# jtaghia/ciMRGP

Hardware: AMD Instinct MI355X
Metric: GP posteriors/sec at N=8192 (Gram + Cholesky + solve + predictive mean/var) (higher is better)
Workload: dtype f64; 1 GPU; BASELINE configs[1]: 1-D, N=8192 single-resolution single-partition RBF GP per GPU, q=2 outputs, N/4=2048 test points, ell=0.1, sf2=1, noise=0.01; partitions_per_gpu=1, backend=none, rows_queues=2, front_queue=True

## Files before the change

### cimrgp_amd/csrc/gemm_nt.hip

```cpp
#include "common.hpp"
#include "gemm_tile.hpp"

namespace cimrgp {

namespace {

template <typename T, bool LOWER, int W>
__global__ __launch_bounds__(256, 2)
void k_gemm_nt_sub(T* __restrict__ C, int64_t ldc,
                   const T* __restrict__ A, int64_t lda,
                   const T* __restrict__ B, int64_t ldb,
                   int M, int N, int K, int tiles_n, int64_t sc, int64_t sa, int64_t sb, int skip_first)
{
    if (skip_first && blockIdx.x == 0) return;
    constexpr int GT = 32 * W;
    __shared__ __attribute__((aligned(16))) unsigned char smem[4 * GT * LROW];
    C += (int64_t)blockIdx.y * sc;
    A += (int64_t)blockIdx.y * sa;
    B += (int64_t)blockIdx.y * sb;
    int ti, tj;
    if (LOWER) {
        const int id = blockIdx.x;
        ti = (int)((sqrtf(8.0f * (float)id + 1.0f) - 1.0f) * 0.5f);
        while (ti * (ti + 1) / 2 > id) --ti;
        while ((ti + 1) * (ti + 2) / 2 <= id) ++ti;
        tj = id - ti * (ti + 1) / 2;
    } else {
        ti = blockIdx.x / tiles_n;
        tj = blockIdx.x - ti * tiles_n;
    }
    const bool interior = (ti + 1) * GT <= M && (tj + 1) * GT <= N && (K % (KT_BYTES / (int)sizeof(T))) == 0;
    if (interior) gemm_tile<T, LOWER, false, W>(smem, C, ldc, A, lda, B, ldb, M, N, K, ti, tj);
    else          gemm_tile<T, LOWER, true,  W>(smem, C, ldc, A, lda, B, ldb, M, N, K, ti, tj);
}


constexpr int PERS_STRIP = 4;

static __device__ __forceinline__ int pers_div(int q, int d)
{
    int r = (int)((float)q / (float)d);
    r -= (r * d > q);
    r += ((r + 1) * d <= q);
    return r;
}

template <bool LOWER>
static __device__ __forceinline__ void pers_tile_decode(int q, int tiles_m, int tiles_n, int& ti, int& tj)
{
    if (LOWER) {
        static_assert(PERS_STRIP == 4, "closed form below");
        const int sfull = tiles_m >> 2;
        int s, h;
        if (q < 8 * sfull * sfull + 2 * sfull) {
            s = (int)((sqrtf(8.0f * (float)q + 1.0f) - 1.0f) * 0.125f);
            s -= (8 * s * s + 2 * s > q);
            s += (8 * (s + 1) * (s + 1) + 2 * (s + 1) <= q);
            h = 4;
        } else {
            s = sfull;
            h = tiles_m - 4 * sfull;
        }
        const int r0 = 4 * s;
        const int off = q - (8 * s * s + 2 * s);
        if (off < h * r0) {
            tj = (h == 4) ? (off >> 2) : (h == 2) ? (off >> 1) : (h == 1) ? off : (int)(((unsigned)off * 43691u) >> 17);
            ti = r0 + off - tj * h;
        } else {
            int o2 = off - h * r0, c = 0;
            if (o2 >= h) {
                o2 -= h; c = 1;
                if (o2 >= h - 1) {
                    o2 -= h - 1; c = 2;
                    if (o2 >= h - 2) { o2 -= h - 2; c = 3; }
                }
            }
            tj = r0 + c;
            ti = r0 + c + o2;
        }
    } else {
        const int per_strip = PERS_STRIP * tiles_n;
        const int s = pers_div(q, per_strip);
        const int r0 = PERS_STRIP * s;
        const int h = min(PERS_STRIP, tiles_m - r0);
        const int off = q - s * per_strip;
        tj = (h == 4) ? (off >> 2) : (h == 2) ? (off >> 1) : (h == 1) ? off : pers_div(off, 3);
        ti = r0 + off - tj * h;
    }
}

static __device__ __forceinline__ void pers_tile_decode_head_first(int q, int tiles_m, int& ti, int& tj)
{
    if (q < tiles_m - 1) { ti = q + 1; tj = 0; return; }
    q -= tiles_m - 1;
    if (q < tiles_m - 1) { ti = q + 1; tj = 1; return; }
    q -= tiles_m - 1;
    pers_tile_decode<true>(q, tiles_m - 2, 0, ti, tj);
    ti += 2;
    tj += 2;
}

static __device__ __forceinline__ int pers_tile_number(int w, int i, int grid, int ntiles)
{
    const int per_xcd = grid >> 3;
    const int x = w & 7, j = w >> 3;
    const int q = (i * 8 + x) * per_xcd + j;
    return q < ntiles ? q : -1;
}

static __device__ __forceinline__ __amdgpu_buffer_rsrc_t tile_rsrc(const void* p)
{
    return __builtin_amdgcn_make_buffer_rsrc(const_cast<void*>(p), 0, 0x7fffffff, 0x00020000);
}
static __device__ __forceinline__ __amdgpu_buffer_rsrc_t tile_rsrc_null(const void* p)
{
    return __builtin_amdgcn_make_buffer_rsrc(const_cast<void*>(p), 0, 0, 0x00020000);
}
typedef unsigned int cbuf_u2 __attribute__((ext_vector_type(2)));
template <typename T> static __device__ __forceinline__ T cbuf_load(__amdgpu_buffer_rsrc_t r, int voff, int soff);
template <> __device__ __forceinline__ double cbuf_load<double>(__amdgpu_buffer_rsrc_t r, int voff, int soff)
{
    const cbuf_u2 v = __builtin_amdgcn_raw_buffer_load_b64(r, voff, soff, 0);
    return __hiloint2double((int)v.y, (int)v.x);
}
template <> __device__ __forceinline__ float cbuf_load<float>(__amdgpu_buffer_rsrc_t r, int voff, int soff)
{
    return __uint_as_float(__builtin_amdgcn_raw_buffer_load_b32(r, voff, soff, 0));
}
template <typename T> static __device__ __forceinline__ void cbuf_store(T v, __amdgpu_buffer_rsrc_t r, int voff, int soff);
template <> __device__ __forceinline__ void cbuf_store<double>(double v, __amdgpu_buffer_rsrc_t r, int voff, int soff)
{
    const cbuf_u2 u = {(unsigned)__double2loint(v), (unsigned)__double2hiint(v)};
    __builtin_amdgcn_raw_buffer_store_b64(u, r, voff, soff, 0);
}
template <> __device__ __forceinline__ void cbuf_store<float>(float v, __amdgpu_buffer_rsrc_t r, int voff, int soff)
{
    __builtin_amdgcn_raw_buffer_store_b32(__float_as_uint(v), r, voff, soff, 0);
}

constexpr int PERS_THREADS = 512;
constexpr int PERS_STAGES = 16;

template <typename T, bool LOWER, int NKT, bool MULTI = false>
__global__ __launch_bounds__(PERS_THREADS)
void k_gemm_nt_pers(T* __restrict__ C, int64_t ldc, const T* __restrict__ A, int64_t lda,
                    const T* __restrict__ B, int64_t ldb, int tiles_m, int tiles_n, int ntiles, int heads, int* __restrict__ flag,
                    int nkc)
{
    static_assert(NKT == 16 || NKT == 8, "sixteen C events per tile: one or two per K stage");
    constexpr int EVS = 16 / NKT;
    using X = Mx<T>;
    using acc_t = typename X::acc_t;
    constexpr int BKE = KT_BYTES / (int)sizeof(T);
    constexpr int GT = 128;
    constexpr int OP_BYTES = GT * LROW;
    constexpr int RS = (sizeof(T) == 8) ? 4 : 1;
    __shared__ __attribute__((aligned(16))) unsigned char smem[4 * OP_BYTES];

    const int tid = threadIdx.x, lane = tid & 63;
    const int wave = __builtin_amdgcn_readfirstlane(tid >> 6);
    const int wr = wave >> 2, wc = wave & 3;
    const int sc = tid & 7, sr = tid >> 3;
    const int grid = (int)gridDim.x, wg = (int)blockIdx.x;

    int a_off_e[2], b_off_e[2];
#pragma unroll
    for (int p = 0; p < 2; ++p) {
        a_off_e[p] = (sr + 64 * p) * (int)lda + sc * X::EPC;
        b_off_e[p] = (sr + 64 * p) * (int)ldb + sc * X::EPC;
    }
    const int frow = lane & 15, fslot = lane >> 4;
    const unsigned a_frag = (unsigned)((wr * 64 + frow) * LROW + fslot * 8);
    const unsigned b_frag = (unsigned)((wc * 32 + frow) * LROW + fslot * 8);
    const int lrow0 = wr * 64 + X::crow(lane, 0), lcol0 = wc * 32 + (lane & 15);
    const int coff = lrow0 * (int)ldc + lcol0;
    const int cbyte0 = coff * (int)sizeof(T);
    const int row_bytes = (int)ldc * (int)sizeof(T);

    auto decode = [&](int q, int& i_, int& j_) {
        if (LOWER && heads > 0) pers_tile_decode_head_first(q, tiles_m, i_, j_);
        else pers_tile_decode<LOWER>(q, tiles_m, tiles_n, i_, j_);
    };
    auto signal_stored = [&]() {
        asm volatile("s_waitcnt vmcnt(0)" ::: "memory");
        __syncthreads();
        if (tid == 0) {
            __builtin_amdgcn_fence(__ATOMIC_RELEASE, "agent");
            asm volatile("s_waitcnt vmcnt(0)" ::: "memory");
            __hip_atomic_fetch_add(flag, 1, __ATOMIC_RELAXED, __HIP_MEMORY_SCOPE_AGENT);
        }
    };
    __shared__ int flag_a[8], flag_b[8];
    if (tid < 8) { flag_a[tid] = -1; flag_b[tid] = -1; }
    int gstage = 0;
#define PERS_POST(flag_)  do { __atomic_signal_fence(__ATOMIC_SEQ_CST);                                                  \
                               __hip_atomic_store(&flag_[wave], gstage, __ATOMIC_RELAXED, __HIP_MEMORY_SCOPE_WORKGROUP);  \
                               __atomic_signal_fence(__ATOMIC_SEQ_CST); } while (0)
#define PERS_PEEK(flag_)  __hip_atomic_load(&flag_[lane & 7], __ATOMIC_RELAXED, __HIP_MEMORY_SCOPE_WORKGROUP)
#define PERS_WAIT(flag_, seen_, g_)                                                                              \
        do {                                                                                                     \
            int v_ = (seen_);                                                                                    \
            while (__builtin_amdgcn_ballot_w64(v_ - (g_) < 0) != 0ull) v_ = PERS_PEEK(flag_);                    \
            __atomic_signal_fence(__ATOMIC_SEQ_CST);                                                             \
        } while (0)
    int it = 0;
    int t = pers_tile_number(wg, it, grid, ntiles);
    if (t < 0) return;
    int ti, tj;
    decode(t, ti, tj);
    int t_nx = pers_tile_number(wg, 1, grid, ntiles), ti_nx = ti, tj_nx = tj;
    if (t_nx >= 0) decode(t_nx, ti_nx, tj_nx);
    bool prev_head = false;
    bool prv_stored = true;
    T* c_cur = C + (int64_t)ti * GT * ldc + (int64_t)tj * GT;
    const T* a_cur = A + (int64_t)ti * GT * lda;
    const T* b_cur = B + (int64_t)tj * GT * ldb;
    T* c_prv = c_cur;
    typedef unsigned int v4u __attribute__((ext_vector_type(4)));
    v4u ra[2], rb[2];
    const v4u sign4 = {0x80000000u, 0x80000000u, 0x80000000u, 0x80000000u};
    uint2 fa[2][4], fb[2][2];
    acc_t acc0[4][2], acc1[4][2];

#define PERS_GLOAD(ap_, bp_, kt_)                                                  \
    {                                                                              \
        _Pragma("unroll") for (int p = 0; p < 2; ++p) {                            \
            ra[p] = *reinterpret_cast<const v4u*>((ap_) + (a_off_e[p] + (kt_) * BKE)); \
            rb[p] = *reinterpret_cast<const v4u*>((bp_) + (b_off_e[p] + (kt_) * BKE)); \
        }                                                                          \
    }
#define PERS_SWRITE(buf_)                                                          \
    {                                                                              \
        unsigned char* as_ = smem + (buf_) * 2 * OP_BYTES;                         \
        unsigned char* bs_ = as_ + OP_BYTES;                                       \
        _Pragma("unroll") for (int p = 0; p < 2; ++p) {                            \
             \
             \
            *reinterpret_cast<v4u*>(as_ + (sr + 64 * p) * LROW + sc * 16) = (sizeof(T) == 4) ? (ra[p] ^ sign4) : ra[p]; \
            *reinterpret_cast<v4u*>(bs_ + (sr + 64 * p) * LROW + sc * 16) = rb[p]; \
        }                                                                          \
    }
#define PERS_FRAGS_NF(set_, buf_, s_)                                              \
    {                                                                              \
        const unsigned char* as_ = smem + (buf_) * 2 * OP_BYTES;                   \
        const unsigned char* bs_ = as_ + OP_BYTES;                                 \
        _Pragma("unroll") for (int mi = 0; mi < 4; ++mi)                           \
            fa[set_][mi] = *reinterpret_cast<const uint2*>(as_ + a_frag + mi * 16 * LROW + (s_) * 32); \
        _Pragma("unroll") for (int ni = 0; ni < 2; ++ni)                           \
            fb[set_][ni] = *reinterpret_cast<const uint2*>(bs_ + b_frag + ni * 16 * LROW + (s_) * 32); \
    }
#define PERS_FRAGS(set_, buf_, s_)  { PERS_FRAGS_NF(set_, buf_, s_) __builtin_amdgcn_sched_barrier(0); }
#define PERS_MMA_NF(cur_, set_)                                                    \
    {                                                                              \
        _Pragma("unroll") for (int mi = 0; mi < 4; ++mi) {                         \
            _Pragma("unroll") for (int ni = 0; ni < 2; ++ni)                       \
                cur_[mi][ni] = (sizeof(T) == 4) ? X::mma(fa[set_][mi], fb[set_][ni], cur_[mi][ni])            \
                                                : X::mma_neg(fa[set_][mi], fb[set_][ni], cur_[mi][ni]);       \
        }                                                                          \
    }
#define PERS_MMA(cur_, set_)  { PERS_MMA_NF(cur_, set_) __builtin_amdgcn_sched_barrier(0); }
#define PERS_INTERLEAVE()                                                          \
    {                                                                              \
        _Pragma("unroll") for (int i_ = 0; i_ < 8; ++i_) {                         \
            __builtin_amdgcn_sched_group_barrier(0x008, 1, 0);                     \
            __builtin_amdgcn_sched_group_barrier(0x096, 6, 0);                     \
        }                                                                          \
        __builtin_amdgcn_sched_barrier(0);                                         \
    }

    PERS_GLOAD(a_cur, b_cur, 0);
#pragma unroll
    for (int mi = 0; mi < 4; ++mi)
#pragma unroll
        for (int ni = 0; ni < 2; ++ni)
#pragma unroll
            for (int r = 0; r < 4; ++r)
                acc0[mi][ni][r] = (c_cur + ((int64_t)(mi * 16 + RS * r) * ldc + ni * 16))[coff];
#pragma unroll
    for (int mi = 0; mi < 4; ++mi)
#pragma unroll
        for (int ni = 0; ni < 2; ++ni) acc1[mi][ni] = acc_zero<T>();
    PERS_SWRITE(0);
    PERS_GLOAD(a_cur, b_cur, 1);
    lds_barrier();
    PERS_FRAGS(0, 0, 0);

#define PERS_EVENT_ONE(oth_, e_)                                                                         \
        {                                                          \
                const int mi_ = (e_) >> 2, ne_ = ((e_) >> 1) & 1, r0_ = 2 * ((e_) & 1);                         \
                 \
                 \
                 \
                const int so0_ = (mi_ * 16 + RS * r0_) * row_bytes + ne_ * 16 * (int)sizeof(T);                 \
                const int so1_ = so0_ + RS * row_bytes;                                                         \
                cbuf_store<T>(oth_[mi_][ne_][r0_], rs_prv, cbyte0, so0_);                                       \
                cbuf_store<T>(oth_[mi_][ne_][r0_ + 1], rs_prv, cbyte0, so1_);                                   \
                              \
                oth_[mi_][ne_][r0_] = cbuf_load<T>(rs_nxt, cbyte0, so0_);                                       \
                oth_[mi_][ne_][r0_ + 1] = cbuf_load<T>(rs_nxt, cbyte0, so1_);                                   \
            }
#define PERS_EVENT_BLOCK(oth_)                                                                                  \
        { _Pragma("unroll") for (int ev_ = 0; ev_ < EVS; ++ev_) { PERS_EVENT_ONE(oth_, kt * EVS + ev_) } }
#define PERS_STAGE_OPERANDS(kt_)                                                                                \
            PERS_SWRITE(((kt_) & 1) ^ 1);                \
            if ((kt_) + 2 < NKT) PERS_GLOAD(a_chk, b_chk, (kt_) + 2)                \
            else                 PERS_GLOAD(a_adv, b_adv, (kt_) + 2 - NKT)
#define PERS_SYNC_TOP()      PERS_WAIT(flag_b, seen_b, gstage - 1);
#define PERS_SYNC_WRITTEN()  PERS_POST(flag_a);
#define PERS_SYNC_READ()     PERS_POST(flag_b); seen_a = PERS_PEEK(flag_a); __builtin_amdgcn_sched_barrier(0);
#define PERS_BARRIER_A()     PERS_WAIT(flag_a, seen_a, gstage)
#define PERS_BARRIER_B()     do { } while (0)
#define PERS_SYNC_PEEK_B()   seen_b = PERS_PEEK(flag_b); __builtin_amdgcn_sched_barrier(0);
#define PERS_SYNC_NEXT()     ++gstage;
#define PERS_PASS(cur_, oth_)                                                                                   \
    {                                                                                                           \
        const int tn_ = t_nx;                                                                                   \
        const bool has_next = tn_ >= 0;                                                                         \
        const int ni_ = has_next ? ti_nx : ti, nj_ = has_next ? tj_nx : tj;                                     \
        const T* c_nxt = C + (int64_t)ni_ * GT * ldc + (int64_t)nj_ * GT;           \
        const __amdgpu_buffer_rsrc_t rs_nxt = tile_rsrc(c_nxt);                                                 \
        const T* a_nxt = A + (int64_t)ni_ * GT * lda;                                                           \
        const T* b_nxt = B + (int64_t)nj_ * GT * ldb;                                                           \
         \
         \
         \
         \
        for (int kc = 0; kc < (MULTI ? nkc : 1); ++kc) {                                                        \
        const bool lastc = !MULTI || (kc + 1 == nkc);                                                           \
        const __amdgpu_buffer_rsrc_t rs_prv = (prv_stored || kc > 0) ? tile_rsrc_null(c_prv) : tile_rsrc(c_prv); \
        const T* a_chk = a_cur + kc * (NKT * BKE);                                                              \
        const T* b_chk = b_cur + kc * (NKT * BKE);                                                              \
        const T* a_adv = lastc ? a_nxt : a_chk + NKT * BKE;                                                     \
        const T* b_adv = lastc ? b_nxt : b_chk + NKT * BKE;                                                     \
        _Pragma("unroll") for (int kt = 0; kt < NKT; ++kt) {                                                    \
            if (kt == NKT / 2 && lastc) {               \
                t_nx = pers_tile_number(wg, it + 2, grid, ntiles);                                              \
                if (t_nx >= 0) decode(t_nx, ti_nx, tj_nx);                                                      \
            }                                                                                                   \
            PERS_SYNC_TOP()                           \
            PERS_STAGE_OPERANDS(kt)                                                                             \
            PERS_SYNC_WRITTEN()                                  \
            PERS_EVENT_BLOCK(oth_)                                                                              \
              \
              \
            PERS_FRAGS_NF(1, kt & 1, 1);                                                                        \
            PERS_MMA_NF(cur_, 0);                                                                               \
            PERS_INTERLEAVE();                                                                                  \
            PERS_FRAGS(0, kt & 1, 2);                                                                           \
            PERS_MMA(cur_, 1);                                                                                  \
            PERS_FRAGS(1, kt & 1, 3);                                                                           \
            PERS_SYNC_READ()                          \
            PERS_MMA(cur_, 0);                                                                                  \
            PERS_BARRIER_A();                                                         \
            PERS_FRAGS(0, (kt & 1) ^ 1, 0);                                  \
            PERS_SYNC_PEEK_B()                        \
            PERS_MMA(cur_, 1);                                                                                  \
            PERS_BARRIER_B();                         \
            PERS_SYNC_NEXT()                                                                                    \
        }                                                                                                       \
        }                                                                                      \
        if (prev_head) signal_stored();               \
        prev_head = (t < heads);                                                                                \
        c_prv = c_cur;                                                                                          \
        if (!has_next) {                                                                                        \
               \
            _Pragma("unroll") for (int mi = 0; mi < 4; ++mi)                                                    \
                _Pragma("unroll") for (int ni = 0; ni < 2; ++ni)                                                \
                    _Pragma("unroll") for (int r = 0; r < 4; ++r)                                               \
                        (c_cur + ((int64_t)(mi * 16 + RS * r) * ldc + ni * 16))[coff] = cur_[mi][ni][r];        \
            if (prev_head) signal_stored();                                                                     \
            return;                                                                                             \
        }                                                                                                       \
        prv_stored = false;                                                                                     \
        t = tn_; ti = ni_; tj = nj_; ++it;                                                                      \
        c_cur = const_cast<T*>(c_nxt); a_cur = a_nxt; b_cur = b_nxt;                                            \
    }

    int seen_a = -1, seen_b = -1;
    for (;;) {
        PERS_PASS(acc0, acc1)
        PERS_PASS(acc1, acc0)
    }
#undef PERS_PASS
#undef PERS_STAGE_OPERANDS
#undef PERS_SYNC_TOP
#undef PERS_SYNC_WRITTEN
#undef PERS_SYNC_READ
#undef PERS_SYNC_PEEK_B
#undef PERS_SYNC_NEXT
#undef PERS_BARRIER_A
#undef PERS_BARRIER_B
#undef PERS_EVENT_BLOCK
#undef PERS_EVENT_ONE
#undef PERS_INTERLEAVE
#undef PERS_MMA
#undef PERS_MMA_NF
#undef PERS_FRAGS_NF
#undef PERS_FRAGS
#undef PERS_SWRITE
#undef PERS_GLOAD
}

constexpr int THIN_RPW = 8;
constexpr int THIN_MAXM = 4;
template <typename T, int M>
__global__ __launch_bounds__(256)
void k_thin_update(T* __restrict__ C, int64_t ldc, const T* __restrict__ A, int64_t lda, const T* __restrict__ B, int64_t ldb,
                   int N, int K, int64_t sc, int64_t sa, int64_t sb)
{
    typedef unsigned int v4u __attribute__((ext_vector_type(4)));
    constexpr int EPL = 32 / (int)sizeof(T);
    constexpr int CH = 64 * EPL;
    C += (int64_t)blockIdx.y * sc;
    A += (int64_t)blockIdx.y * sa;
    B += (int64_t)blockIdx.y * sb;
    const int lane = threadIdx.x & 63, wave = threadIdx.x >> 6;
    const int n0 = ((int)blockIdx.x * 4 + wave) * THIN_RPW;
    if (n0 >= N) return;
    T acc[THIN_RPW][M];
#pragma unroll
    for (int i = 0; i < THIN_RPW; ++i)
#pragma unroll
        for (int r = 0; r < M; ++r) acc[i][r] = (T)0;
    for (int kc = 0; kc < K; kc += CH) {
        const int ke = kc + lane * EPL;
        const bool live = ke < K;
        T av[M][EPL];
#pragma unroll
        for (int r = 0; r < M; ++r) {
            union { v4u v[2]; T t[EPL]; } u;
            u.v[0] = live ? *reinterpret_cast<const v4u*>(A + (int64_t)r * lda + ke) : v4u{0, 0, 0, 0};
            u.v[1] = (live && ke + EPL / 2 < K) ? *reinterpret_cast<const v4u*>(A + (int64_t)r * lda + ke + EPL / 2) : v4u{0, 0, 0, 0};
#pragma unroll
            for (int e = 0; e < EPL; ++e) av[r][e] = u.t[e];
        }
        union { v4u v[2]; T t[EPL]; } bv[THIN_RPW];
#pragma unroll
        for (int i = 0; i < THIN_RPW; ++i) {
            const int n = min(n0 + i, N - 1);
            const T* bp = B + (int64_t)n * ldb + ke;
            bv[i].v[0] = live ? *reinterpret_cast<const v4u*>(bp) : v4u{0, 0, 0, 0};
            bv[i].v[1] = (live && ke + EPL / 2 < K) ? *reinterpret_cast<const v4u*>(bp + EPL / 2) : v4u{0, 0, 0, 0};
        }
#pragma unroll
        for (int i = 0; i < THIN_RPW; ++i)
#pragma unroll
            for (int r = 0; r < M; ++r)
#pragma unroll
                for (int e = 0; e < EPL; ++e) acc[i][r] += av[r][e] * bv[i].t[e];
    }
#pragma unroll
    for (int i = 0; i < THIN_RPW; ++i)
#pragma unroll
        for (int r = 0; r < M; ++r) {
            T v = acc[i][r];
#pragma unroll
            for (int off = 32; off > 0; off >>= 1) v += __shfl_xor(v, off, 64);
            acc[i][r] = v;
        }
    if (lane < THIN_RPW * M) {
        const int i = lane / M, r = lane - i * M;
        T v = (T)0;
#pragma unroll
        for (int ii = 0; ii < THIN_RPW; ++ii)
#pragma unroll
            for (int rr = 0; rr < M; ++rr)
                if (ii == i && rr == r) v = acc[ii][rr];
        if (n0 + i < N) C[(int64_t)r * ldc + n0 + i] -= v;
    }
}

}

template <typename T, int W>
static int gemm_launch(T* c, int64_t ldc, const T* a, int64_t lda, const T* b, int64_t ldb,
                       int64_t m, int64_t n, int k, bool lower, hipStream_t st, const GemmBatch& bt)
{
    const char* fn = "gemm_nt_sub";
    constexpr int GT = 32 * W;
    const int64_t tm = (m + GT - 1) / GT, tn = (n + GT - 1) / GT;
    const int64_t tiles = lower ? tm * (tm + 1) / 2 : tm * tn;
    CIMRGP_REQUIRE(tiles < (1ll << 31), fn, "grid too large");
    CIMRGP_REQUIRE(bt.count >= 1 && bt.count < 65536, fn, "batch count out of range");
    const dim3 grid((unsigned)tiles, (unsigned)bt.count);
    if (lower) hipLaunchKernelGGL((k_gemm_nt_sub<T, true, W>), grid, dim3(256), 0, st,
                                  c, ldc, a, lda, b, ldb, (int)m, (int)n, k, (int)tn, bt.sc, bt.sa, bt.sb, bt.skip_first);
    else       hipLaunchKernelGGL((k_gemm_nt_sub<T, false, W>), grid, dim3(256), 0, st,
                                  c, ldc, a, lda, b, ldb, (int)m, (int)n, k, (int)tn, bt.sc, bt.sa, bt.sb, bt.skip_first);
    CIMRGP_LAUNCH_CHECK(fn);
    return 0;
}

int gemm_pers_head_tiles(int64_t m, int k, int elem_bytes)
{
    if (elem_bytes != 8) return 0;
    const int bke = KT_BYTES / elem_bytes;
    if (knobs().gemm_pers < 8 || m % 128 != 0 || m / 128 < 3 || k % bke != 0 || k / bke != PERS_STAGES) return 0;
    return (int)(2 * (m / 128) - 2);
}

bool gemm_uses_tile64(int64_t m, int64_t n, bool lower, int count)
{
    const int64_t t128 = ((m + 127) / 128) * ((n + 127) / 128) / (lower ? 2 : 1) * count;
    const int64_t t64 = ((m + 63) / 64) * ((n + 63) / 64) / (lower ? 2 : 1) * count;
    const int64_t thin = (m < n) ? m : n;
    return !lower && t64 >= 32 && thin > 32 && (t128 < 768 || thin <= 64);
}

template <typename T>
int gemm_nt_sub(T* c, int64_t ldc, const T* a, int64_t lda, const T* b, int64_t ldb,
                int64_t m, int64_t n, int k, bool lower, hipStream_t st, GemmBatch bt)
{
    const char* fn = "gemm_nt_sub";
    if (m <= 0 || n <= 0 || k <= 0) return 0;
    CIMRGP_REQUIRE(m < (1ll << 30) && n < (1ll << 30), fn, "matrix too large");
    CIMRGP_REQUIRE(aligned16(a) && aligned16(b), fn, "operand base not 16-byte aligned");
    CIMRGP_REQUIRE(lda % Mx<T>::EPC == 0 && ldb % Mx<T>::EPC == 0, fn, "leading dimension not a multiple of 16 bytes");
    CIMRGP_REQUIRE(!lower || m == n, fn, "lower update needs a square C");
    if (!lower && m <= THIN_MAXM && !bt.skip_first && !bt.head_first && k % Mx<T>::EPC == 0 && aligned16(a) && aligned16(b)) {
        const dim3 grid((unsigned)((n + 4 * THIN_RPW - 1) / (4 * THIN_RPW)), (unsigned)bt.count);
#define CIMRGP_THIN(M_) case M_: hipLaunchKernelGGL((k_thin_update<T, M_>), grid, dim3(256), 0, st, c, ldc, a, lda, b, ldb, (int)n, k, bt.sc, bt.sa, bt.sb); break;
        switch ((int)m) { CIMRGP_THIN(1) CIMRGP_THIN(2) CIMRGP_THIN(3) CIMRGP_THIN(4) }
#undef CIMRGP_THIN
        CIMRGP_LAUNCH_CHECK(fn);
        return 0;
    }
    CIMRGP_REQUIRE(!bt.skip_first || gemm_uses_tile64(m, n, lower, bt.count), fn, "skip_first needs a 64-tile launch");
    const int64_t t128 = ((m + 127) / 128) * ((n + 127) / 128) / (lower ? 2 : 1) * bt.count;
    const int64_t t64 = ((m + 63) / 64) * ((n + 63) / 64) / (lower ? 2 : 1) * bt.count;
    if constexpr (sizeof(T) == 8) {
        constexpr int bke = KT_BYTES / (int)sizeof(T);
        const int want = (bt.pers >= 0) ? bt.pers : knobs().gemm_pers;
        const int nkt = (k % bke) ? 0 : k / bke;
        constexpr int pers_nkt = PERS_STAGES;
        const int nkc = (nkt > 0 && nkt % pers_nkt == 0) ? nkt / pers_nkt : 0;
        if (want >= 8 && nkc >= 1 && nkc <= knobs().pers_max_chunks && (nkc == 1 || !bt.head_first) &&
            bt.count == 1 && !bt.skip_first && m % 128 == 0 && n % 128 == 0 &&
            ldc < (1ll << 20) && lda < (1ll << 23) && ldb < (1ll << 23) && (t128 >= knobs().pers_min_tiles || bt.head_first || bt.pers_force)) {
            const int64_t tm = m / 128, tn = n / 128;
            const int heads = (bt.head_first && lower && tm >= 3) ? (int)(2 * tm - 2) : 0;
            CIMRGP_REQUIRE(!bt.head_first || heads > 0, fn, "a head-first update needs a lower update of at least 3 x 3 tiles");
            const int64_t tiles = (lower ? tm * (tm + 1) / 2 : tm * tn) - (heads ? 1 : 0);
            const int cus = (want < 256 ? want : 256) & ~7;
            const int64_t rounds = (tiles + cus - 1) / cus;
            int64_t g8 = (tiles + rounds - 1) / rounds;
            g8 = (g8 + 7) / 8 * 8;
            if (g8 > cus) g8 = cus;
            const dim3 grid((unsigned)g8);
#define CIMRGP_PERS_LAUNCH(LOW_, MULTI_) \
            hipLaunchKernelGGL((k_gemm_nt_pers<T, LOW_, pers_nkt, MULTI_>), grid, dim3(PERS_THREADS), 0, st, c, ldc, a, lda, b, ldb, (int)tm, (int)tn, (int)tiles, heads, bt.flag, nkc)
            if (lower) { if (nkc > 1) CIMRGP_PERS_LAUNCH(true, true); else CIMRGP_PERS_LAUNCH(true, false); }
            else       { if (nkc > 1) CIMRGP_PERS_LAUNCH(false, true); else CIMRGP_PERS_LAUNCH(false, false); }
#undef CIMRGP_PERS_LAUNCH
            CIMRGP_LAUNCH_CHECK(fn);
            return 0;
        }
    }
    CIMRGP_REQUIRE(!bt.head_first, fn, "head-first update not eligible for the persistent kernel (gemm_pers_eligible)");
    const int64_t thin = (m < n) ? m : n;
    if (!bt.skip_first && thin <= 32) return gemm_launch<T, 1>(c, ldc, a, lda, b, ldb, m, n, k, lower, st, bt);
    if (t64 < 32) return gemm_launch<T, 1>(c, ldc, a, lda, b, ldb, m, n, k, lower, st, bt);
    if (t128 < 768 || thin <= 64) return gemm_launch<T, 2>(c, ldc, a, lda, b, ldb, m, n, k, lower, st, bt);
    return gemm_launch<T, 4>(c, ldc, a, lda, b, ldb, m, n, k, lower, st, bt);
}

template int gemm_nt_sub<double>(double*, int64_t, const double*, int64_t, const double*, int64_t,
                                 int64_t, int64_t, int, bool, hipStream_t, GemmBatch);
template int gemm_nt_sub<float>(float*, int64_t, const float*, int64_t, const float*, int64_t,
                                int64_t, int64_t, int, bool, hipStream_t, GemmBatch);

}
```

Baseline: 147.8 posteriors/s.

## Partition persistent GEMM tiles into contiguous per-XCD regions and stream C traffic

Tile scheduling for the persistent GEMM kernel moves into a shared header. The assignment changes from interleaving tiles round-robin across the eight XCDs to giving each XCD a contiguous range of tiles: column-major rectangular regions for the general case, and head tiles first then contiguous ranges for the lower case. This should keep A/B panel reuse inside each XCD's L2. C loads and stores in the single-chunk case now carry a streaming cache-policy bit so C traffic does not evict operands. A guard on tile count is added for the general path to avoid int overflow in the new index math.

New measurement: 148.5 posteriors/s (median of 6 runs). Within noise of the previous version (+0.5%).

```diff
diff --git a/cimrgp_amd/csrc/gemm_nt.hip b/cimrgp_amd/csrc/gemm_nt.hip
--- a/cimrgp_amd/csrc/gemm_nt.hip
+++ b/cimrgp_amd/csrc/gemm_nt.hip
@@ -1,5 +1,6 @@
 #include "common.hpp"
 #include "gemm_tile.hpp"
+#include "pers_order.hpp"
 
 namespace cimrgp {
 
@@ -35,107 +36,33 @@
 }
 
 
-constexpr int PERS_STRIP = 4;
-
-static __device__ __forceinline__ int pers_div(int q, int d)
-{
-    int r = (int)((float)q / (float)d);
-    r -= (r * d > q);
-    r += ((r + 1) * d <= q);
-    return r;
-}
-
-template <bool LOWER>
-static __device__ __forceinline__ void pers_tile_decode(int q, int tiles_m, int tiles_n, int& ti, int& tj)
-{
-    if (LOWER) {
-        static_assert(PERS_STRIP == 4, "closed form below");
-        const int sfull = tiles_m >> 2;
-        int s, h;
-        if (q < 8 * sfull * sfull + 2 * sfull) {
-            s = (int)((sqrtf(8.0f * (float)q + 1.0f) - 1.0f) * 0.125f);
-            s -= (8 * s * s + 2 * s > q);
-            s += (8 * (s + 1) * (s + 1) + 2 * (s + 1) <= q);
-            h = 4;
-        } else {
-            s = sfull;
-            h = tiles_m - 4 * sfull;
-        }
-        const int r0 = 4 * s;
-        const int off = q - (8 * s * s + 2 * s);
-        if (off < h * r0) {
-            tj = (h == 4) ? (off >> 2) : (h == 2) ? (off >> 1) : (h == 1) ? off : (int)(((unsigned)off * 43691u) >> 17);
-            ti = r0 + off - tj * h;
-        } else {
-            int o2 = off - h * r0, c = 0;
-            if (o2 >= h) {
-                o2 -= h; c = 1;
-                if (o2 >= h - 1) {
-                    o2 -= h - 1; c = 2;
-                    if (o2 >= h - 2) { o2 -= h - 2; c = 3; }
-                }
-            }
-            tj = r0 + c;
-            ti = r0 + c + o2;
-        }
+static __device__ __forceinline__ __amdgpu_buffer_rsrc_t tile_rsrc(const void* p)
+{
+    return __builtin_amdgcn_make_buffer_rsrc(const_cast<void*>(p), 0, 0x7fffffff, 0x00020000);
+}
+static __device__ __forceinline__ __amdgpu_buffer_rsrc_t tile_rsrc_null(const void* p)
+{
+    return __builtin_amdgcn_make_buffer_rsrc(const_cast<void*>(p), 0, 0, 0x00020000);
+}
+constexpr int PERS_C_STREAM = 2;
+typedef unsigned int cbuf_u2 __attribute__((ext_vector_type(2)));
+template <typename T, int AUX> static __device__ __forceinline__ T cbuf_load(__amdgpu_buffer_rsrc_t r, int voff, int soff)
+{
+    if constexpr (sizeof(T) == 8) {
+        const cbuf_u2 v = __builtin_amdgcn_raw_buffer_load_b64(r, voff, soff, AUX);
+        return __hiloint2double((int)v.y, (int)v.x);
     } else {
-        const int per_strip = PERS_STRIP * tiles_n;
-        const int s = pers_div(q, per_strip);
-        const int r0 = PERS_STRIP * s;
-        const int h = min(PERS_STRIP, tiles_m - r0);
-        const int off = q - s * per_strip;
-        tj = (h == 4) ? (off >> 2) : (h == 2) ? (off >> 1) : (h == 1) ? off : pers_div(off, 3);
-        ti = r0 + off - tj * h;
-    }
-}
-
-static __device__ __forceinline__ void pers_tile_decode_head_first(int q, int tiles_m, int& ti, int& tj)
-{
-    if (q < tiles_m - 1) { ti = q + 1; tj = 0; return; }
-    q -= tiles_m - 1;
-    if (q < tiles_m - 1) { ti = q + 1; tj = 1; return; }
-    q -= tiles_m - 1;
-    pers_tile_decode<true>(q, tiles_m - 2, 0, ti, tj);
-    ti += 2;
-    tj += 2;
-}
-
-static __device__ __forceinline__ int pers_tile_number(int w, int i, int grid, int ntiles)
-{
-    const int per_xcd = grid >> 3;
-    const int x = w & 7, j = w >> 3;
-    const int q = (i * 8 + x) * per_xcd + j;
-    return q < ntiles ? q : -1;
-}
-
-static __device__ __forceinline__ __amdgpu_buffer_rsrc_t tile_rsrc(const void* p)
-{
-    return __builtin_amdgcn_make_buffer_rsrc(const_cast<void*>(p), 0, 0x7fffffff, 0x00020000);
-}
-static __device__ __forceinline__ __amdgpu_buffer_rsrc_t tile_rsrc_null(const void* p)
-{
-    return __builtin_amdgcn_make_buffer_rsrc(const_cast<void*>(p), 0, 0, 0x00020000);
-}
-typedef unsigned int cbuf_u2 __attribute__((ext_vector_type(2)));
-template <typename T> static __device__ __forceinline__ T cbuf_load(__amdgpu_buffer_rsrc_t r, int voff, int soff);
-template <> __device__ __forceinline__ double cbuf_load<double>(__amdgpu_buffer_rsrc_t r, int voff, int soff)
-{
-    const cbuf_u2 v = __builtin_amdgcn_raw_buffer_load_b64(r, voff, soff, 0);
-    return __hiloint2double((int)v.y, (int)v.x);
-}
-template <> __device__ __forceinline__ float cbuf_load<float>(__amdgpu_buffer_rsrc_t r, int voff, int soff)
-{
-    return __uint_as_float(__builtin_amdgcn_raw_buffer_load_b32(r, voff, soff, 0));
-}
-template <typename T> static __device__ __forceinline__ void cbuf_store(T v, __amdgpu_buffer_rsrc_t r, int voff, int soff);
-template <> __device__ __forceinline__ void cbuf_store<double>(double v, __amdgpu_buffer_rsrc_t r, int voff, int soff)
-{
-    const cbuf_u2 u = {(unsigned)__double2loint(v), (unsigned)__double2hiint(v)};
-    __builtin_amdgcn_raw_buffer_store_b64(u, r, voff, soff, 0);
-}
-template <> __device__ __forceinline__ void cbuf_store<float>(float v, __amdgpu_buffer_rsrc_t r, int voff, int soff)
-{
-    __builtin_amdgcn_raw_buffer_store_b32(__float_as_uint(v), r, voff, soff, 0);
+        return __uint_as_float(__builtin_amdgcn_raw_buffer_load_b32(r, voff, soff, AUX));
+    }
+}
+template <typename T, int AUX> static __device__ __forceinline__ void cbuf_store(T v, __amdgpu_buffer_rsrc_t r, int voff, int soff)
+{
+    if constexpr (sizeof(T) == 8) {
+        const cbuf_u2 u = {(unsigned)__double2loint(v), (unsigned)__double2hiint(v)};
+        __builtin_amdgcn_raw_buffer_store_b64(u, r, voff, soff, AUX);
+    } else {
+        __builtin_amdgcn_raw_buffer_store_b32(__float_as_uint(v), r, voff, soff, AUX);
+    }
 }
 
 constexpr int PERS_THREADS = 512;
@@ -149,6 +76,7 @@
 {
     static_assert(NKT == 16 || NKT == 8, "sixteen C events per tile: one or two per K stage");
     constexpr int EVS = 16 / NKT;
+    constexpr int CAUX = MULTI ? 0 : PERS_C_STREAM;
     using X = Mx<T>;
     using acc_t = typename X::acc_t;
     constexpr int BKE = KT_BYTES / (int)sizeof(T);
@@ -204,11 +132,11 @@
             __atomic_signal_fence(__ATOMIC_SEQ_CST);                                                             \
         } while (0)
     int it = 0;
-    int t = pers_tile_number(wg, it, grid, ntiles);
+    int t = pers_tile_number<LOWER>(wg, it, grid, ntiles, heads, tiles_m);
     if (t < 0) return;
     int ti, tj;
     decode(t, ti, tj);
-    int t_nx = pers_tile_number(wg, 1, grid, ntiles), ti_nx = ti, tj_nx = tj;
+    int t_nx = pers_tile_number<LOWER>(wg, 1, grid, ntiles, heads, tiles_m), ti_nx = ti, tj_nx = tj;
     if (t_nx >= 0) decode(t_nx, ti_nx, tj_nx);
     bool prev_head = false;
     bool prv_stored = true;
@@ -293,11 +221,11 @@
                  \
                 const int so0_ = (mi_ * 16 + RS * r0_) * row_bytes + ne_ * 16 * (int)sizeof(T);                 \
                 const int so1_ = so0_ + RS * row_bytes;                                                         \
-                cbuf_store<T>(oth_[mi_][ne_][r0_], rs_prv, cbyte0, so0_);                                       \
-                cbuf_store<T>(oth_[mi_][ne_][r0_ + 1], rs_prv, cbyte0, so1_);                                   \
+                cbuf_store<T, CAUX>(oth_[mi_][ne_][r0_], rs_prv, cbyte0, so0_);                                 \
+                cbuf_store<T, CAUX>(oth_[mi_][ne_][r0_ + 1], rs_prv, cbyte0, so1_);                             \
                               \
-                oth_[mi_][ne_][r0_] = cbuf_load<T>(rs_nxt, cbyte0, so0_);                                       \
-                oth_[mi_][ne_][r0_ + 1] = cbuf_load<T>(rs_nxt, cbyte0, so1_);                                   \
+                oth_[mi_][ne_][r0_] = cbuf_load<T, CAUX>(rs_nxt, cbyte0, so0_);                                 \
+                oth_[mi_][ne_][r0_ + 1] = cbuf_load<T, CAUX>(rs_nxt, cbyte0, so1_);                             \
             }
 #define PERS_EVENT_BLOCK(oth_)                                                                                  \
         { _Pragma("unroll") for (int ev_ = 0; ev_ < EVS; ++ev_) { PERS_EVENT_ONE(oth_, kt * EVS + ev_) } }
@@ -334,7 +262,7 @@
         const T* b_adv = lastc ? b_nxt : b_chk + NKT * BKE;                                                     \
         _Pragma("unroll") for (int kt = 0; kt < NKT; ++kt) {                                                    \
             if (kt == NKT / 2 && lastc) {               \
-                t_nx = pers_tile_number(wg, it + 2, grid, ntiles);                                              \
+                t_nx = pers_tile_number<LOWER>(wg, it + 2, grid, ntiles, heads, tiles_m);                                             \
                 if (t_nx >= 0) decode(t_nx, ti_nx, tj_nx);                                                      \
             }                                                                                                   \
             PERS_SYNC_TOP()                           \
@@ -535,7 +463,7 @@
         constexpr int pers_nkt = PERS_STAGES;
         const int nkc = (nkt > 0 && nkt % pers_nkt == 0) ? nkt / pers_nkt : 0;
         if (want >= 8 && nkc >= 1 && nkc <= knobs().pers_max_chunks && (nkc == 1 || !bt.head_first) &&
-            bt.count == 1 && !bt.skip_first && m % 128 == 0 && n % 128 == 0 &&
+            bt.count == 1 && !bt.skip_first && m % 128 == 0 && n % 128 == 0 && (lower || (m / 128) * (n / 128) < (1 << 19)) &&
             ldc < (1ll << 20) && lda < (1ll << 23) && ldb < (1ll << 23) && (t128 >= knobs().pers_min_tiles || bt.head_first || bt.pers_force)) {
             const int64_t tm = m / 128, tn = n / 128;
             const int heads = (bt.head_first && lower && tm >= 3) ? (int)(2 * tm - 2) : 0;
diff --git a/cimrgp_amd/csrc/pers_order.hpp b/cimrgp_amd/csrc/pers_order.hpp
--- /dev/null
+++ b/cimrgp_amd/csrc/pers_order.hpp
@@ -0,0 +1,110 @@
+#pragma once
+#include <cmath>
+
+#if defined(__HIPCC__) || defined(__CUDACC__)
+#define PERS_HD __host__ __device__ __forceinline__
+#else
+#define PERS_HD inline
+#endif
+
+namespace cimrgp {
+
+constexpr int PERS_STRIP = 4;
+
+static PERS_HD int pers_div(int q, int d)
+{
+    int r = (int)((float)q / (float)d);
+    r -= (r * d > q);
+    r += ((r + 1) * d <= q);
+    return r;
+}
+
+template <bool LOWER>
+static PERS_HD void pers_tile_decode(int q, int tiles_m, int tiles_n, int& ti, int& tj)
+{
+    if (LOWER) {
+        static_assert(PERS_STRIP == 4, "closed form below");
+        const int sfull = tiles_m >> 2;
+        int s, h;
+        if (q < 8 * sfull * sfull + 2 * sfull) {
+            s = (int)((sqrtf(8.0f * (float)q + 1.0f) - 1.0f) * 0.125f);
+            s -= (8 * s * s + 2 * s > q);
+            s += (8 * (s + 1) * (s + 1) + 2 * (s + 1) <= q);
+            h = 4;
+        } else {
+            s = sfull;
+            h = tiles_m - 4 * sfull;
+        }
+        const int r0 = 4 * s;
+        const int off = q - (8 * s * s + 2 * s);
+        if (off < h * r0) {
+            tj = (h == 4) ? (off >> 2) : (h == 2) ? (off >> 1) : (h == 1) ? off : (int)(((unsigned)off * 43691u) >> 17);
+            ti = r0 + off - tj * h;
+        } else {
+            int o2 = off - h * r0, c = 0;
+            if (o2 >= h) {
+                o2 -= h; c = 1;
+                if (o2 >= h - 1) {
+                    o2 -= h - 1; c = 2;
+                    if (o2 >= h - 2) { o2 -= h - 2; c = 3; }
+                }
+            }
+            tj = r0 + c;
+            ti = r0 + c + o2;
+        }
+    } else {
+        tj = pers_div(q, tiles_m);
+        ti = q - tj * tiles_m;
+    }
+}
+
+static PERS_HD void pers_tile_decode_head_first(int q, int tiles_m, int& ti, int& tj)
+{
+    if (q < tiles_m - 1) { ti = q + 1; tj = 0; return; }
+    q -= tiles_m - 1;
+    if (q < tiles_m - 1) { ti = q + 1; tj = 1; return; }
+    q -= tiles_m - 1;
+    pers_tile_decode<true>(q, tiles_m - 2, 0, ti, tj);
+    ti += 2;
+    tj += 2;
+}
+
+template <bool LOWER>
+static PERS_HD int pers_tile_number(int w, int i, int grid, int ntiles, int heads, int tiles_m)
+{
+    const int per_xcd = grid >> 3;
+    const int x = w & 7, j = w >> 3;
+    const int p = i * per_xcd + j;
+    if (!LOWER) {
+        const int s = (x * ntiles) >> 3, e = ((x + 1) * ntiles) >> 3;
+        if (p >= e - s) return -1;
+        const int ca = pers_div(s, tiles_m), ra = s - ca * tiles_m;
+        const int cb = pers_div(e, tiles_m), rb = e - cb * tiles_m;
+        const int wn = cb - ca;
+        const int lo = ra < rb ? ra : rb, hi = ra < rb ? rb : ra;
+        const int wmid = wn + (ra < rb ? 1 : -1);
+        const int flo = lo * wn, fhi = flo + (hi - lo) * wmid;
+        int r, fr;
+        if (p < flo)      { r = pers_div(p, wn);                    fr = r * wn; }
+        else if (p < fhi) { r = lo + pers_div(p - flo, wmid);       fr = flo + (r - lo) * wmid; }
+        else              { r = hi + pers_div(p - fhi, wn);                  fr = fhi + (r - hi) * wn; }
+        const int c = ca + (r < ra) + (p - fr);
+        return c * tiles_m + r;
+    }
+    const int hx = (heads - x + 7) >> 3;
+    if (p < hx) return x + 8 * p;
+    const int nrem = ntiles - heads;
+    const int hq = heads >> 3, hr = heads & 7;
+    int start, end;
+    if (nrem < 8) {
+        start = (x * nrem) >> 3;
+        end = ((x + 1) * nrem) >> 3;
+    } else {
+        start = ((x * ntiles) >> 3) - (hq * x + (x < hr ? x : hr));
+        end = (((x + 1) * ntiles) >> 3) - (hq * (x + 1) + (x + 1 < hr ? x + 1 : hr));
+    }
+    const int r = start + (p - hx);
+    return r < end ? heads + r : -1;
+}
+
+}
```
